# iamsonderr/icl-mixed-precision-gmres

Hardware: AMD Instinct MI355X
Metric: GMRES iterations/sec + SpMV achieved HBM GB/s, 10M-nnz CSR, 1/2/4/8 GPUs (higher is better)
Workload: dtype f32; 1 GPU; BAND banded CSR n=1000000, offsets -5..+4, nnz=9999975 (1e6 rows = 10M nnz per GPU, 1 GPU(s)); GMRES(30) mixed (fp32 Arnoldi, f32 accumulation, fp64 residual/update), cgs, identity preconditioner, tol=0; step=one restart cycle = 30 iterations, rows_per_gpu=1000000, nnz=9999975, parallelism=one GPU

## Files before the change

### icl-mixed-precision-gmres_amd/__init__.py

```python
from __future__ import annotations

import ctypes as C
import os
import subprocess
from dataclasses import dataclass, field
from pathlib import Path
from typing import Optional

import numpy as np

from ._abi import (ACCUMS, ENGINES, MODES, ORTHS, PRECS, SPMV_FORMATS, STATUS, ArnoldiDesc, CondestResult, CyclePolicy, HostCsr, RankLayout, SolveArgs,
                   SolveResult, condest_args, condest_dict)

PKG_DIR = Path(__file__).resolve().parent
REPO_DIR = PKG_DIR.parent
LIB_DIR = PKG_DIR / "lib"
HIP_LIB = LIB_DIR / "libmpgmres_hip.so"
HOST_LIB = LIB_DIR / "libmpgmres_host.so"
CLI = PKG_DIR / "bin" / "gmres_perf_test"


def build(jobs: int = 8) -> None:
    subprocess.run(["make", "-C", str(PKG_DIR), f"-j{jobs}"], check=True)

# ... 128 lines not shown
    lib.mpg_halo_recv_count.argtypes = [C.c_void_p, _I32]
    lib.mpg_halo_recv_count.restype = _I32
    lib.mpg_halo_recv_rows.argtypes = [C.c_void_p, _I32, P64]
    lib.mpg_halo_set_send.argtypes = [C.c_void_p, _I32, _I32, P64]
    lib.mpg_halo_local_cols.argtypes = [C.c_void_p, P32]
    lib.mpg_halo_free.argtypes = [C.c_void_p]
    lib.mpg_halo_free.restype = None
    lib.mpg_rccl_unique_id.argtypes = [C.c_char_p, C.c_int]
    lib.mpg_engine_create_dist.argtypes = [C.POINTER(SolveArgs), C.c_void_p, C.c_char_p, _I32, _I32,
                                           C.POINTER(C.c_void_p), C.c_char_p, C.c_int]
    lib.mpg_solve_loopback.argtypes = [C.POINTER(SolveArgs), _I32, C.POINTER(SolveResult)]
    lib.mpg_solve_loopback_ex.argtypes = [C.POINTER(SolveArgs), _I32, C.POINTER(SolveResult), C.c_void_p]
    lib.mpg_solve_multi_gpu.argtypes = [C.POINTER(SolveArgs), _I32, C.c_void_p, C.POINTER(SolveResult), C.c_void_p]
    lib.mpg_engine_comm_ranks.argtypes = [C.c_void_p]
    lib.mpg_engine_sell_columns.argtypes = [C.c_void_p, C.POINTER(C.c_int32), C.POINTER(C.c_int64),
                                            C.POINTER(C.c_int64)]
    lib.mpg_engine_half_stats.argtypes = [C.c_void_p, C.POINTER(C.c_int64)]
    lib.mpg_engine_slices_per_wave.argtypes = [C.c_void_p]
    lib.mpg_engine_givens_folded.argtypes = [C.c_void_p]
    lib.mpg_engine_step_dots_steps.argtypes = [C.c_void_p]
    lib.mpg_engine_step_dots_status.argtypes = [C.c_void_p, C.c_int]
    lib.mpg_engine_givens_rider.argtypes = [C.c_void_p]
    lib.mpg_engine_cgs_stream_steps.argtypes = [C.c_void_p]
    lib.mpg_engine_tail_fold.argtypes = [C.c_void_p]
    lib.mpg_engine_cycle_policy.argtypes = [C.c_void_p, C.POINTER(CyclePolicy)]
    lib.mpg_cycle_plan_describe.argtypes = [C.POINTER(CyclePolicy), C.c_char_p, C.c_int]
    lib.mpg_engine_accum.argtypes = [C.c_void_p]
    lib.mpg_engine_basis.argtypes = [C.c_void_p]
    lib.mpg_engine_prec_fused.argtypes = [C.c_void_p]
    lib.mpg_engine_prec_sweeps.argtypes = [C.c_void_p]
    lib.mpg_engine_prec_interval.argtypes = [C.c_void_p, C.POINTER(C.c_double), C.POINTER(C.c_double)]
    lib.mpg_cheb_coeffs.argtypes = [C.c_int, C.c_double, C.c_double, C.POINTER(C.c_double), C.POINTER(C.c_double)]
    lib.mpg_engine_prec_roots.argtypes = [C.c_void_p, C.POINTER(C.c_double), C.POINTER(C.c_double), C.c_int32]
    lib.mpg_gmres_poly_roots.argtypes = [C.c_int, C.POINTER(C.c_double), C.c_int, C.POINTER(C.c_double),
                                         C.POINTER(C.c_double), C.POINTER(C.c_int)]
    lib.mpg_engine_prologue_format.argtypes = [C.c_void_p]
    lib.mpg_engine_sell_shared_slices.argtypes = [C.c_void_p]
    lib.mpg_engine_sell_shared_slices.restype = C.c_int64
    lib.mpg_engine_sell_sigma.argtypes = [C.c_void_p]
    lib.mpg_solve_from.argtypes = [C.POINTER(SolveArgs), C.c_void_p, C.POINTER(SolveResult)]
    lib.mpg_solve_from.restype = C.c_int
    lib.mpg_engine_rearm.argtypes = [C.c_void_p, C.c_void_p, C.c_void_p, C.c_void_p, C.c_int]
    lib.mpg_engine_x.argtypes = [C.c_void_p, C.c_void_p, C.c_int]
    lib.mpg_engine_solves.argtypes = [C.c_void_p]
    lib.mpg_engine_graph_captures.argtypes = [C.c_void_p]

# ... 774 lines not shown
        per = (C.c_double * cap)()
        which = {"spmv": 0, "cgs_update": 2, "dots": 3}[phase]
        cnt = self._lib.mpg_engine_time_phase_stamps(self._h, which, reps, C.byref(ms), per, cap)
        if cnt < 0:
            msg = self._lib.mpg_engine_last_error(self._h).decode(errors="replace")
            raise RuntimeError(f"mpg_engine_time_phase_stamps failed ({cnt}): {msg}")
        return ms.value, [per[i] for i in range(min(cnt, cap))]

    def phase_bytes(self, phase: str) -> float:
        return float(self._lib.mpg_engine_phase_bytes(self._h, self.PHASES[phase]))

    def spmv_layout(self) -> dict:
        f, w, cb, st, win = C.c_int32(), C.c_int32(), C.c_int32(), C.c_int64(), C.c_int32()
        if self._lib.mpg_engine_spmv_layout(self._h, C.byref(f), C.byref(w), C.byref(cb), C.byref(st), C.byref(win)):
            raise RuntimeError("mpg_engine_spmv_layout failed")
        fused = int(self._lib.mpg_engine_step_dots_steps(self._h))
        pf = int(self._lib.mpg_engine_prec_fused(self._h))
        ps = int(self._lib.mpg_engine_prec_sweeps(self._h))
        ia, ib = C.c_double(), C.c_double()
        has_iv = self._lib.mpg_engine_prec_interval(self._h, C.byref(ia), C.byref(ib)) == 0
        rre, rim = (C.c_double * 64)(), (C.c_double * 64)()
        nroots = int(self._lib.mpg_engine_prec_roots(self._h, rre, rim, 64))
        stream = int(self._lib.mpg_engine_cgs_stream_steps(self._h))
        rider = int(self._lib.mpg_engine_givens_rider(self._h)) == 1
        tail = int(self._lib.mpg_engine_tail_fold(self._h)) == 1
        basis = int(self._lib.mpg_engine_basis(self._h))
        return _Layout({**({"dots_fused": fused} if fused > 0 else {}), **({"givens_rider": True} if rider else {}),
                **({"tail_fold": True} if tail else {}),
                **({"cgs_stream": stream} if stream > 0 else {}), "format": {1: "csr", 2: "sell", 3: "node"}[f.value], "vec_width": w.value, "col_bytes": cb.value,
                "stored": st.value, "window": bool(win.value),
                "slices_per_wave": int(self._lib.mpg_engine_slices_per_wave(self._h)),
                "givens_folded": bool(self._lib.mpg_engine_givens_folded(self._h) == 1),
                "accum": {0: "f64", 1: "f32"}[int(self._lib.mpg_engine_accum(self._h))],
                **({"basis": {1: "f16", 2: "f16emu"}[basis]} if basis else {}),
                **({"prec_fused": pf} if pf >= 0 else {}),
                **({"prec_sweeps": ps} if ps >= 0 else {}),
                **({"prec_interval": (ia.value, ib.value)} if has_iv else {}),
                **({"prec_roots": [complex(rre[i], rim[i]) for i in range(nroots)]} if nroots >= 0 else {}),
                "prologue": {1: "csr", 2: "sell", 3: "node"}[int(self._lib.mpg_engine_prologue_format(self._h))]})

    def step_dots_status(self, k: int) -> int:
        return int(self._lib.mpg_engine_step_dots_status(self._h, k))

    def cycle_policy(self) -> CyclePolicy:
        p = CyclePolicy()
        if self._lib.mpg_engine_cycle_policy(self._h, C.byref(p)):
            raise RuntimeError("mpg_engine_cycle_policy failed")
        return p

    def sell_columns(self) -> dict:
# ... 28 lines not shown
```

### icl-mixed-precision-gmres_amd/csrc/arnoldi.hip

```cpp
#include "arnoldi_launch.hpp"

#include <cstdlib>
#include <new>
#include <algorithm>
#include <vector>

using namespace mpg;

namespace {

int64_t sell_copy_bytes(const mpg_arnoldi* a);

void node_prologue_build(mpg_arnoldi* a) {
    const char* e = std::getenv("MPG_NODE_PROLOGUE");
    if ((e && *e == '0') || a->node.nblk == 0 || a->d.n_front != 0 || a->d.outer_type != MPG_F64) return;
    if (hipMalloc((void**)&a->rsum, (size_t)std::max(a->d.n, 1) * sizeof(double)) != hipSuccess) {
        (void)hipGetLastError();
        return;
    }
    if (a->d.val_outer == a->d.val_inner && a->d.inner_val == MPG_F64) {
        a->node_res = &a->node;
        return;
    }
    const int64_t csr = a->d.A->nnz * 12 + ((int64_t)a->d.n + 1) * 4;
// ... 52 lines not shown
}

}

extern "C" {

int mpg_arnoldi_create(mpg_ctx_t ctx, const mpg_arnoldi_desc* desc, mpg_arnoldi_t* out) {
    if (!ctx || !desc || !out || !desc->A || desc->n < 0 || desc->n_ext < desc->n || desc->m < 1 ||
        desc->m > 1000 || desc->orth < 0 || desc->orth > 2)
        return MPG_ERR_ARG;
    *out = nullptr;
    int combo = combo_of(*desc);
    if (combo < 0) return MPG_ERR_UNSUPPORTED;
    if (desc->A->rows != desc->n || desc->A->cols > desc->n_ext) return MPG_ERR_ARG;
    if (desc->inner_row_exp && desc->inner_val != MPG_F16) return MPG_ERR_ARG;
    if (desc->block_dinv && (desc->jacobi || desc->prec_block < 2 || desc->prec_block > 4)) return MPG_ERR_ARG;
    mpg_arnoldi* a = new (std::nothrow) mpg_arnoldi();
    if (!a) return MPG_ERR_ALLOC;
    a->ctx = ctx;
    a->d = *desc;
    a->combo = combo;
    a->tsize = desc->vec_type == MPG_F64 ? 8 : 4;
    if (const char* e = std::getenv("MPG_CGS_PREFETCH"); e && (*e == '0' || *e == '1')) a->cgs_pref = *e - '0';
    a->G = desc->A->nblocks < kGroups ? (desc->A->nblocks > 0 ? desc->A->nblocks : 1) : kGroups;
    a->Grb = desc->A->nblocks > 0 ? desc->A->nblocks : 1;
    a->Gd = (int)std::min<int64_t>(kCombineGroups, std::max<int64_t>(1, ((int64_t)desc->n + 4 * kCombineBlock - 1) /
                                                                          (4 * kCombineBlock)));
    if (desc->n_front < 0) {
        delete a;
        return MPG_ERR_ARG;
    }
    a->front = MPG_FRONT_PAD(desc->n_front);
    const size_t align = 256 / a->tsize;
    a->ld = ((int64_t)desc->n + align - 1) / align * align;
    if (a->ld == 0) a->ld = align;
    const int m = desc->m;
    auto alloc = [&](void** p, size_t bytes) {
        if (hipMalloc(p, bytes ? bytes : 16) != hipSuccess) return false;
        return hipMemsetAsync(*p, 0, bytes ? bytes : 16, ctx->stream) == hipSuccess;
    };
    bool ok = alloc(&a->V, (size_t)a->ld * (m + 1) * a->tsize) && alloc(&a->H, (size_t)(m + 1) * m * a->tsize) &&
              alloc(&a->small, (size_t)7 * (m + 1) * a->tsize) &&
              alloc(&a->wbase[0], (size_t)(a->front + desc->n_ext + 64) * a->tsize) &&
              alloc(&a->wbase[1], (size_t)(a->front + desc->n_ext + 64) * a->tsize) &&
              alloc((void**)&a->partial, std::max<size_t>(std::max<size_t>((size_t)(kNC + 4) * a->Grb,
                                                                           (size_t)(m + 4) * a->G),
// ... 188 lines not shown
        else
            k_prologue_finish_parts<T, X, 1024><<<1, 1024, 0, a->ctx->stream>>>(
                a->last_G, a->last_part, a->sums, m, static_cast<T*>(a->s()), static_cast<T*>(a->inv()), a->report,
                stage, hcol);
        return MPG_OK;
    });
    if (st) return st;
    a->tail_staged = false;
    MPG_LAUNCH_CHECK(a->ctx);
    return MPG_OK;
}

int mpg_arnoldi_reduce(mpg_arnoldi_t a, int ncols) { return phases(a).reduce(a, ncols); }

int mpg_arnoldi_spmv(mpg_arnoldi_t a, int k) { return phases(a).spmv(a, k, 0, false); }
int mpg_arnoldi_spmv_dots(mpg_arnoldi_t a, int k, int fold) {
    if (fold < 0 || fold > 2) return MPG_ERR_ARG;
    return phases(a).spmv(a, k, fold, true);
}
int mpg_arnoldi_spmv_dots_supported(mpg_arnoldi_t a, int k) { return phases(a).spmv_dots_ok(a, k); }
int mpg_arnoldi_step_dots(mpg_arnoldi_t a, int k, int fold) { return phases(a).step_dots(a, k, fold); }
int mpg_arnoldi_step_dots_supported(mpg_arnoldi_t a, int k) { return phases(a).step_dots_ok(a, k); }
int mpg_arnoldi_cgs_stream_at(mpg_arnoldi_t a, int k) { return phases(a).cgs_stream_at(a, k); }
int mpg_arnoldi_givens_spmv(mpg_arnoldi_t a, int k) { return phases(a).spmv(a, k, 1, false); }
int mpg_arnoldi_givens_partials_spmv(mpg_arnoldi_t a, int k) { return phases(a).spmv(a, k, 2, false); }
int mpg_arnoldi_fold_max_m(void) { return kFoldMaxM; }
int mpg_arnoldi_partials_max_cols(void) { return kWideMax; }

constexpr int kFoldMaxGroups = 4096;
int mpg_arnoldi_fold_pays(mpg_arnoldi_t a) {
    if (!a) return 0;
    const char* env = std::getenv("MPG_FOLD_MAX_GROUPS");
    const int64_t limit = env && *env ? std::atoll(env) : kFoldMaxGroups;
    if (a->node.nblk > 0) {
        const int tpw = node_tpw(a->node);
        return (a->node.ntiles + tpw - 1) / tpw <= limit ? 1 : 0;
    }
    const SellCopy& S = a->sell;
    if (S.nslices == 0) return a->Grb <= limit ? 1 : 0;
    const int per_group = (kStepSellBlock / kWave) * (sell_uniform(S) && sell_pair(S) ? 2 : 1);
    return (S.nslices + per_group - 1) / per_group <= limit ? 1 : 0;
}

int mpg_arnoldi_dots(mpg_arnoldi_t a, int k) { return phases(a).dots(a, k, false); }
int mpg_arnoldi_dots_sums(mpg_arnoldi_t a, int k) { return phases(a).dots(a, k, true); }

// ... 110 lines not shown
```

### icl-mixed-precision-gmres_amd/csrc/arnoldi_dots.hpp

```cpp
#pragma once

#include "arnoldi_spmv.hpp"

namespace {

template <class T, int BS = kBlock, bool COMBINE = false, class A = double>
__global__ __launch_bounds__(BS) void k_panel_dots(int n, const T* __restrict__ V, int64_t ld, int c0, int nc,
                                                   const T* __restrict__ w, double* __restrict__ partial,
                                                   unsigned* __restrict__ cnt, double* __restrict__ sums) {
    A acc[kNC];
#pragma unroll
    for (int c = 0; c < kNC; ++c) acc[c] = A(0);
    const int n4 = n & ~3;
    const T* __restrict__ Vb = V + (int64_t)c0 * ld;
    for (int i = 4 * (blockIdx.x * BS + threadIdx.x); i < n4; i += 4 * gridDim.x * BS) {
        A wv[4];
        Row4<T>::load(w + i, wv);
#pragma unroll
        for (int c = 0; c < kNC; ++c) {
            if (c < nc) {
                A v[4];
                Row4<T>::load(Vb + (int64_t)c * ld + i, v);
                acc[c] += v[0] * wv[0] + v[1] * wv[1] + v[2] * wv[2] + v[3] * wv[3];
            }
        }
// ... 64 lines not shown
        }
    }
    store_partials<NP, BS>(acc, NC, partial, G);
}

template <class T, int BS, int NC, class A = double, class BT = T>
__device__ __forceinline__ void dots_panel(int n, const typename Basis<T, BT>::elem* __restrict__ V, int64_t ld,
                                           const T* __restrict__ w, double* __restrict__ partial) {
    dots_panel_from<T, BS, NC, A, BT>(n, V, ld, DotsGlobal<T, A, BT>{w, {}}, partial);
}

template <class T, int BS, int NC, bool STAMP = false, class AT = double>
__global__ __launch_bounds__(BS) void k_dots_nc(int n, const T* __restrict__ V, int64_t ld,
                                                const T* __restrict__ w, double* __restrict__ partial,
                                                unsigned long long* stamp) {
    using A = typename AccOf<AT>::type;
    using Bs = BasisOf<T, AT>;
    stamp_at<STAMP>(stamp, 0);
    dots_panel<T, BS, NC, A, typename AccOf<AT>::template basis<T>>(n, basis_ptr<Bs>(V), ld, w, partial);
    stamp_at<STAMP>(stamp, 1);
}

constexpr int kStepDotsRows = 4 * kCombineBlock;

template <class T, class A, int HELD>
struct DotsStaged {
    static constexpr bool kStaged = true;
    static constexpr int kHeld = HELD;
    const T* wst;
    const T* vkst;
    int base;
    Raw4<T> held[HELD > 0 ? HELD : 1];
    __device__ __forceinline__ void load_w(int i, A (&wv)[4]) const { Row4<T>::load(wst + (i - base), wv); }
    __device__ __forceinline__ Raw4<T> newest(int i) const {
        Raw4<T> r;
        r.load(vkst + (i - base));
        return r;
    }
};

__device__ __forceinline__ void wave_lds_handoff() {
    __atomic_signal_fence(__ATOMIC_SEQ_CST);
    __builtin_amdgcn_s_waitcnt(0xC07F);
    wave_lds_sync();
    __atomic_signal_fence(__ATOMIC_SEQ_CST);
}

template <class T, class P, int W, bool FOLD, int BE, int NC, bool PF, class A>
__global__ __launch_bounds__(kCombineBlock) void k_step_dots(int n, int nslices, const int16_t* __restrict__ col,
                                                             const T* __restrict__ val, const T* __restrict__ wprev,
                                                             const T* __restrict__ inv_p, T* __restrict__ V,
                                                             int64_t ld, int k, const P* __restrict__ diag,
                                                             T* __restrict__ w, GivensFold<T> fold,
                                                             const int32_t* __restrict__ spat,
                                                             const int64_t* __restrict__ coff,
                                                             const int16_t* __restrict__ pat, int64_t ustride,
                                                             double* __restrict__ dpart) {
    static_assert(std::is_same_v<T, float>, "fp32 basis and values");
    using CI = int16_t;
    using Row = SellRow<T, CI, W, (MPG_SELL_NT != 0), BE>;
    constexpr int BS = kCombineBlock, SPW = 4, NW = BS / kWave;
    constexpr int RB = kStepDotsRows, RW = SPW * kWave;
    constexpr int WL = kWinLo + RW + kWinHi;
    static_assert(NW * RW == RB, "four slices per wave cover the workgroup's rows");
    static_assert(RW == 4 * kWave, "a wave's slices are its lanes' row groups of dots_panel_from");
    __shared__ __attribute__((aligned(16))) T win[NW][WL];
    __shared__ __attribute__((aligned(16))) T wst[RB];
    const int tid = threadIdx.x, lane = tid & (kWave - 1), wid = wave_id();
    constexpr int NG = kBlock / kWave;
    if constexpr (FOLD) {
        if (blockIdx.x == gridDim.x - 1) {
// ... 20 lines not shown
    if constexpr (FOLD) fold_parts_load(fold, lane, part);
    __builtin_amdgcn_sched_barrier(0);
    const int i4 = base + 4 * tid;
    const bool in4 = i4 < n;
    Raw4<T> wr;
    wr.load(wprev + (in4 ? i4 : 0));
    const int clo = row0 - kWinLo + lane, chi = row0 + RW + lane;
    const bool lo_in = clo >= 0 && clo < n, hi_in = chi < n;
    const T wlo = wprev[lo_in ? clo : 0];
    const T whi = wprev[hi_in ? chi : 0];
    __builtin_amdgcn_sched_barrier(0);
#pragma unroll
    for (int p = 0; p < SPW; ++p) {
        row[p].init_vals(lane, val);
        row[p].load_vals(0);
    }
    __builtin_amdgcn_sched_barrier(0);
#pragma unroll
    for (int p = 0; p < SPW; ++p) {
        row[p].init_finish(lane, col, val, nullptr, pat);
        row[p].load_cols(0);
    }
    __builtin_amdgcn_sched_barrier(0);
    constexpr int B = kColBatch<T>;
    constexpr int HMAX = FOLD ? 6 : B;
    constexpr int HELD = !PF ? 0 : NC - 1 < HMAX ? NC - 1 : HMAX;
    T* const wwin = win[wid];
    DotsStaged<T, A, HELD> src;
    src.wst = wst + wid * RW;
    src.vkst = wwin + kWinLo;
    src.base = row0;
    if constexpr (HELD > 0) {
#pragma unroll
        for (int u = 0; u < HELD; ++u) src.held[u].load(V + (int64_t)u * ld + (in4 ? i4 : 0));
    }
    __builtin_amdgcn_sched_barrier(0);
    T inv;
    if constexpr (FOLD) inv = inv_of_norm2<T>(fold_parts_sum(fold, part));
    else inv = *inv_p;
    {
        T vq[4];
#pragma unroll
        for (int r = 0; r < 4; ++r) vq[r] = in4 ? (T)(wr.template at<T>(r) * inv) : T(0);
        Row4<T>::store(wwin + kWinLo + 4 * lane, vq);
        wwin[lane] = lo_in ? (T)(wlo * inv) : T(0);
        wwin[kWinLo + RW + lane] = hi_in ? (T)(whi * inv) : T(0);
    }
    wave_lds_handoff();
    auto xv = [&](int c) { return (double)wwin[c - row0 + kWinLo]; };
    A sum[SPW] = {};
#pragma unroll
    for (int p = 0; p < SPW; ++p)
        if (live_p[p]) row[p].sum(0, xv, sum[p]);
#pragma unroll
    for (int p = 0; p < SPW; ++p) {
        if (live_p[p])
            for (int q = Row::U; q < row[p].steps; q += Row::U) {
                row[p].load(q);
                row[p].sum(q, xv, sum[p]);
            }
        const int i = (s0 + p) * kWave + lane;
        T wi = T(0);
        if (live_p[p] && i < n) {
            const T t = (T)sum[p];
            wi = precond<T, P>(t, diag, i);
            w[i] = wi;
            V[(int64_t)k * ld + i] = wwin[i - row0 + kWinLo];
        }
        wst[i - base] = wi;
    }
    wave_lds_handoff();
    dots_panel_from<T, BS, NC, A>(n, V, ld, src, dpart, G);
}

template <class T, int BS, int NCL, class A = double>
__global__ __launch_bounds__(BS) void k_dots_panels(int n, const T* __restrict__ V, int64_t ld,
                                                    const T* __restrict__ w, double* __restrict__ partial) {
    const int c0 = blockIdx.y * kNC;
    double* __restrict__ part = partial + (size_t)c0 * gridDim.x;
    if (blockIdx.y + 1 < gridDim.y) dots_panel<T, BS, kNC, A>(n, V + (int64_t)c0 * ld, ld, w, part);
    else dots_panel<T, BS, NCL, A>(n, V + (int64_t)c0 * ld, ld, w, part);
}

}
```

### icl-mixed-precision-gmres_amd/csrc/arnoldi_launch.hpp

```cpp
#pragma once

#include "arnoldi_dots.hpp"
#include "arnoldi_orth.hpp"
#include "arnoldi_update.hpp"

#include <algorithm>
#include <cstdlib>
#include <tuple>
#include <type_traits>

namespace {

template <class A, class F>
int dispatch_acc(int combo, F&& f) {
    if constexpr (std::is_same_v<A, double>) {
        return dispatch(combo, f);
    } else {
        switch (combo) {
            case 2: return f(float(), float(), float(), float());
            case 3: return f(float(), double(), float(), float());
            case 4: return f(float(), double(), float(), half_v());
            default: return MPG_ERR_UNSUPPORTED;
        }
    }
// ... 195 lines not shown
    if (st) return st;
    if (dots) {
        a->last_G = a->fd_ng;
        a->last_part = a->dpart;
    }
    MPG_LAUNCH_CHECK(a->ctx);
    return MPG_OK;
}

template <class A>
int step_dots_check(const mpg_arnoldi* a, int k) {
    if (!a || k < 0 || k >= a->d.m) return MPG_ERR_ARG;
    const SellCopy& S = a->sell;
    const bool ok = std::is_same_v<A, float> && (a->combo == 2 || a->combo == 3) && plain_basis(a) &&
                    a->d.orth != kOrthMGS && a->d.orth != kOrthCGSR && k + 1 <= kNC &&
                    a->d.n > 0 && a->d.n % 4 == 0 &&
                    (int64_t)a->Gd * kStepDotsRows >= a->d.n &&
                    a->front == 0 && a->d.n_ext == a->d.n &&
                    S.nslices > 0 && S.c16 && S.win && !S.rows && sell_uniform(S) && S.W == 2 &&
                    S.ustride / kWave <= 10;
    return ok ? MPG_OK : MPG_ERR_UNSUPPORTED;
}

template <class A>
int step_dots_run(mpg_arnoldi_t a, int k, int fold) {
    if (!a || k < 0 || k >= a->d.m || fold < 0 || fold > 2) return MPG_ERR_ARG;
    if (int st = step_dots_check<A>(a, k)) return st;
    if (fold && (k < 1 || a->d.m > kFoldMaxM)) return MPG_ERR_ARG;
    if constexpr (std::is_same_v<A, float>) {
        using T = float;
        using P = float;
        const bool again = fold == 2 && a->sd_k == k && a->last_part == a->dpart;
        if (fold == 2 && !again) {
            a->sd_k = k;
            a->sd_part = a->last_part;
            a->sd_G = a->last_G;
        }
        if (fold == 2 && (a->sd_G > kBlock || a->sd_part == a->dpart)) return MPG_ERR_ARG;
        GivensFold<T> gf{nullptr, 0, {}};
        if (fold) gf = GivensFold<T>{fold == 2 ? a->sd_part : a->sums, fold == 2 ? a->sd_G : 0, givens_args<T>(a, k - 1)};
        const SellCopy& S = a->sell;
        const P* diag = a->d.jacobi ? static_cast<const P*>(a->d.diag) : nullptr;
        int st = with_nc<kNC>(k + 1, [&](auto nc) {
            constexpr int NC = decltype(nc)::value;
            return with_flag(fold, [&](auto fo) {
                launch_timed(a->ctx, k_step_dots<T, P, 2, decltype(fo)::value, 10, NC, true, A>,
                             dim3(a->Gd + (fold ? 1 : 0)), dim3(kCombineBlock), a->d.n, S.nslices,
                             static_cast<const int16_t*>(S.col), static_cast<const T*>(S.val),
                             static_cast<const T*>(a->w[k & 1]), static_cast<const T*>(a->inv()),
                             static_cast<T*>(a->V), a->ld, k, diag, static_cast<T*>(a->w[(k + 1) & 1]), gf, S.spat,
                             S.coff, static_cast<const int16_t*>(S.pat), S.ustride, a->dpart);
                return (int)MPG_OK;
            });
        });
        if (st) return st;
        a->last_G = a->Gd;
        a->last_part = a->dpart;
        MPG_LAUNCH_CHECK(a->ctx);
        return MPG_OK;
    } else {
        return MPG_ERR_UNSUPPORTED;
    }
}

inline int wide_groups(const mpg_arnoldi* a, int ncols) {
    const int np = (ncols + kNC - 1) / kNC;
    return std::max(1, std::min(a->Gd, kCombineGroups / np));
}

inline unsigned long long* take_stamp(mpg_arnoldi* a, int64_t waves) {
    unsigned long long* p = a->ctx->stamp_next;
    a->ctx->stamp_next = nullptr;
    return p && waves <= a->ctx->stamp_cap ? p : nullptr;
}

// ... 314 lines not shown
                constexpr bool SNAP = decltype(snap)::value;
                k_update_tail_nc<T, X, decltype(nc)::value, A, stream, SNAP><<<a->Gd, kCombineBlock, 0, a->ctx->stream>>>(
                    a->d.n, static_cast<const T*>(a->V), a->ld, static_cast<X*>(a->d.x),
                    SNAP ? static_cast<X*>(a->x_snap) : nullptr, tl);
                return (int)MPG_OK;
            });
        });
    });
    if (st) return st;
    a->tail_staged = true;
    MPG_LAUNCH_CHECK(a->ctx);
    return MPG_OK;
}

}

struct mpg_arnoldi_phases {
    int (*reduce)(mpg_arnoldi* a, int ncols);
    int (*spmv)(mpg_arnoldi* a, int k, int fold, bool dots);
    int (*step_dots)(mpg_arnoldi* a, int k, int fold);
    int (*step_dots_ok)(const mpg_arnoldi* a, int k);
    int (*spmv_dots_ok)(const mpg_arnoldi* a, int k);
    int (*cgs_stream_at)(const mpg_arnoldi* a, int k);
    int (*dots)(mpg_arnoldi* a, int k, bool combine);
    int (*cgs)(mpg_arnoldi* a, int k, int pass, bool givens, bool from_partials, bool no_next);
    int (*mgs)(mpg_arnoldi* a, int k, int j, bool from_partials);
    int (*givens)(mpg_arnoldi* a, int k, bool from_partials);
    int (*update)(mpg_arnoldi* a, int k);
    int (*update_tail)(mpg_arnoldi* a, int m, int flags);
};
__attribute__((visibility("hidden"))) const mpg_arnoldi_phases& mpg_arnoldi_phases_acc32();

namespace {
template <class A>
mpg_arnoldi_phases phases_of() {
    return {reduce_run<A>, spmv_run<A>,     step_dots_run<A>, step_dots_check<A>, spmv_dots_check<A>, cgs_stream_check<A>,
            dots_run<A>,   cgs_run<A>,      mgs_run<A>,       givens_run<A>,      update_run<A>,      update_tail_run<A>};
}
}
```

### icl-mixed-precision-gmres_amd/csrc/arnoldi_plan.hpp

```cpp
#pragma once

#include "internal.hpp"
#include "node_tile.hpp"
#include "sell_tile.hpp"
#include "mpgmres/arnoldi.h"

#include <algorithm>
#include <cstdlib>
#include <type_traits>

using namespace mpg;

namespace {

constexpr int kNC = 32;
constexpr int kGroups = 1024;
constexpr int kCombineBlock = 1024;
constexpr int kCombineGroups = 256;
constexpr int kOrthMGS = 1, kOrthCGSR = 2;
constexpr int kFoldMaxM = 128;
constexpr int kWideMax = 128;

template <int C, int N, class F>
__device__ __forceinline__ void static_for(F&& f) {
// ... 33 lines not shown
struct mpg_arnoldi {
    mpg_ctx* ctx = nullptr;
    mpg_arnoldi_desc d{};
    int combo = 0;
    int G = 1;
    int Grb = 1;
    int last_G = 1;
    double* last_part = nullptr;
    int64_t ld = 0;
    size_t tsize = 8;
    void* V = nullptr;
    void* H = nullptr;
    void* small = nullptr;
    void* w[2] = {nullptr, nullptr};
    void* wbase[2] = {nullptr, nullptr};
    int front = 0;
    double* partial = nullptr;
    double* dpart = nullptr;
    double* sums = nullptr;
    double* report = nullptr;
    unsigned* counters = nullptr;
    int Gd = 1;
    int cgs_pref = -1;
    SellCopy sell;
    SellCopy sell_outer;
    NodeCopy node;
    NodeCopy node_outer;
    const NodeCopy* node_res = nullptr;
    double* rsum = nullptr;
    bool outer_is_inner = false;
    double* fd_part = nullptr;
    unsigned* fd_cnt = nullptr;
    int fd_gs = 0, fd_ng = 0;
    int sd_k = -1, sd_G = 0;
    double* sd_part = nullptr;
    bool acc32 = false;
    int basis = 0;
    void* x_snap = nullptr;
    bool tail_staged = false;

    char* small_at(int slot) const { return static_cast<char*>(small) + (size_t)slot * (d.m + 1) * tsize; }
    void* cs() const { return small_at(0); }
    void* sn() const { return small_at(1); }
    void* s() const { return small_at(2); }
    void* corr() const { return small_at(3); }
    void* inv() const { return small_at(4); }
// ... 50 lines not shown
```

### icl-mixed-precision-gmres_amd/csrc/lds_ring.hpp

```cpp
#pragma once

#include "internal.hpp"

namespace {

typedef __attribute__((address_space(3))) void* lds_ptr_t;
typedef float f32x4_t __attribute__((ext_vector_type(4)));
constexpr int kStreamSlots = 9;

__device__ __forceinline__ double cgs_stream_load_partial(const double* p) {
    double v;
    asm volatile("global_load_dwordx2 %0, %1, off" : "=v"(v) : "v"(p) : "memory");
    return v;
}
template <int BEHIND>
__device__ __forceinline__ void cgs_stream_wait_partials(double (&p)[8]) {
    asm volatile("s_waitcnt vmcnt(%8)"
                 : "+v"(p[0]), "+v"(p[1]), "+v"(p[2]), "+v"(p[3]), "+v"(p[4]), "+v"(p[5]), "+v"(p[6]), "+v"(p[7])
                 : "i"(BEHIND)
                 : "memory");
    __builtin_amdgcn_sched_barrier(0);
}
template <int BEHIND>
__device__ __forceinline__ void cgs_stream_take(unsigned slot_lds, unsigned coef_lds, f32x4_t& v, float& cu) {
    asm volatile("s_waitcnt vmcnt(%4)\n\tds_read_b128 %0, %2\n\tds_read_b32 %1, %3\n\ts_waitcnt lgkmcnt(0)"
                 : "=&v"(v), "=&v"(cu)
                 : "v"(slot_lds), "v"(coef_lds), "i"(BEHIND)
                 : "memory");
    __builtin_amdgcn_sched_barrier(0);
}
__device__ __forceinline__ void cgs_stream_request(const float* g, unsigned lds_wave) {
    __builtin_amdgcn_global_load_lds(g, (lds_ptr_t)(size_t)lds_wave, 16, 0, 0);
}
__device__ __forceinline__ void cgs_stream_pin(float (&t)[4]) {
    asm volatile("" : "+v"(t[0]), "+v"(t[1]), "+v"(t[2]), "+v"(t[3]));
}

}
```

### icl-mixed-precision-gmres_amd/host/fused_gmres.cpp

```cpp
#include "fused_gmres.hpp"

#include <algorithm>
#include <chrono>
#include <cmath>
#include <cstdio>
#include <cstring>
#include <functional>
#include <stdexcept>
#include <thread>

#include "gmres.hpp"
#include "types_hip.hpp"

namespace mpg {

DevMem::DevMem(mpg_ctx_t c, size_t b) : ctx(c), bytes(b) { check(mpg_malloc(c, b, &p), "mpg_malloc", c); }
DevMem::~DevMem() {
    if (p) mpg_free(ctx, p);
}
DevMem& DevMem::operator=(DevMem&& o) noexcept {
    if (this != &o) {
        if (p) mpg_free(ctx, p);
        ctx = o.ctx;
        p = o.p;
// ... 1013 lines not shown
    }
    return p_->poly_roots.count;
}
bool FusedEngine::prec_interval(double* a, double* b) const {
    if (!p_->cheb) return false;
    if (a) *a = p_->cheb_iv.a;
    if (b) *b = p_->cheb_iv.b;
    return true;
}
int FusedEngine::step_dots_steps() const {
    return (int)std::count_if(p_->cycle.begin(), p_->cycle.end(), [](const Op& o) { return o.kind == OpKind::StepDots; });
}
bool FusedEngine::givens_rider() const {
    return std::any_of(p_->cycle.begin(), p_->cycle.end(), [](const Op& o) { return o.kind == OpKind::StepDots && o.b != 0; });
}
bool FusedEngine::tail_fold() const {
    return std::any_of(p_->cycle.begin(), p_->cycle.end(), [](const Op& o) { return o.kind == OpKind::GivensUpdate; });
}
int FusedEngine::cgs_stream_steps() const {
    return (int)std::count_if(p_->cycle.begin(), p_->cycle.end(), [&](const Op& o) {
        return o.kind == OpKind::CgsPartials && mpg_arnoldi_cgs_stream_at(p_->arn, o.a) == 1;
    });
}
const CyclePolicy& FusedEngine::policy() const { return p_->pol; }
const std::vector<Op>& FusedEngine::cycle_ops() const { return p_->cycle; }
hipStream_t FusedEngine::stream() const { return p_->stream(); }
mpg_ctx_t FusedEngine::ctx() const { return p_->ctx; }

void fill_history(const FusedEngine& e, mpg_solve_result* r) {
    r->status = e.status;
    r->restarts = e.restarts;
    r->inner_k = e.inner_k;
    r->total_iters = (int64_t)e.total_iters();
    r->minvb_norm = e.minvb_norm;
    r->setup_seconds = e.setup_seconds;
    r->n_cycles = (int64_t)e.cycles.size();
    for (size_t c = 0; c < e.cycles.size() && (int64_t)c < r->cycle_cap; ++c) {
        if (r->cyc_r_norm) r->cyc_r_norm[c] = e.cycles[c].r_norm;
        if (r->cyc_normalization) r->cyc_normalization[c] = e.cycles[c].normalization;
        if (r->cyc_beta) r->cyc_beta[c] = e.cycles[c].beta;
    }
    r->nonfinite_steps = e.breakdown.steps;
    r->nonfinite_cycles = e.breakdown.cycles;
    r->first_nonfinite_step = e.breakdown.first_step;
    r->n_steps = (int64_t)e.step_res.size();
    for (size_t s = 0; s < e.step_res.size() && (int64_t)s < r->step_cap; ++s) {
// ... 129 lines not shown
int mpg_engine_prologue_format(mpg_engine_t e) {
    if (!e || !e->eng) return MPG_ERR_ARG;
    return mpg_arnoldi_prologue_format(e->eng->arnoldi());
}

int mpg_engine_givens_folded(mpg_engine_t e) {
    if (!e || !e->eng) return MPG_ERR_ARG;
    return e->eng->policy().fold;
}

int mpg_engine_step_dots_steps(mpg_engine_t e) {
    if (!e || !e->eng) return MPG_ERR_ARG;
    return e->eng->step_dots_steps();
}

int mpg_engine_givens_rider(mpg_engine_t e) {
    if (!e || !e->eng) return MPG_ERR_ARG;
    return e->eng->givens_rider() ? 1 : 0;
}

int mpg_engine_tail_fold(mpg_engine_t e) {
    return e && e->eng ? (e->eng->tail_fold() ? 1 : 0) : -1;
}
int mpg_engine_cgs_stream_steps(mpg_engine_t e) {
    if (!e || !e->eng) return MPG_ERR_ARG;
    return e->eng->cgs_stream_steps();
}

int mpg_engine_cycle_policy(mpg_engine_t e, mpg_cycle_policy* out) {
    if (!e || !e->eng || !out) return MPG_ERR_ARG;
    *out = e->eng->policy();
    return MPG_OK;
}

int mpg_engine_step_dots_status(mpg_engine_t e, int k) {
    if (!e || !e->eng) return MPG_ERR_ARG;
    return mpg_arnoldi_step_dots_supported(e->eng->arnoldi(), k);
}

int mpg_engine_comm_ranks(mpg_engine_t e) {
    if (!e || !e->eng) return MPG_ERR_ARG;
    return e->comm ? e->comm->transport_ranks() : 1;
}

int64_t mpg_engine_sell_shared_slices(mpg_engine_t e) {
    if (!e || !e->eng) return MPG_ERR_ARG;
// ... 35 lines not shown
```

### icl-mixed-precision-gmres_amd/host/fused_gmres.hpp

```cpp
#ifndef MPGMRES_FUSED_GMRES_HPP
#define MPGMRES_FUSED_GMRES_HPP

#include <hip/hip_runtime.h>

#include <functional>
#include <memory>
#include <stdexcept>
#include <string>
#include <vector>

#include "IterUtil.hpp"
#include "cycle_plan.hpp"
#include "mpgmres/arnoldi.h"
#include "mpgmres/capi.h"
#include "mpgmres/solve.h"
#include "types_hip.hpp"

namespace mpg {

inline void check_sweep_prec_args(const mpg_solve_args& a, const std::string& name) {
    if (a.jacobi_steps < 1 || a.jacobi_steps > 64)
        throw std::invalid_argument("prec " + name + ": jacobi_steps = " + std::to_string(a.jacobi_steps) +
                                    " is outside [1, 64]");
    if (a.mode == MPG_MODE_SINGLE_PREC)
// ... 70 lines not shown

    int run(int max_cycles, bool& done);
    void finish_report(mpg_solve_result* r);

    void rearm(const double* b, const double* x0, const double* x_true, int flags);
    void copy_x(double* dst, bool dst_on_device);
    int solves() const { return solves_; }
    int graph_captures() const { return graph_captures_; }

    size_t total_iters() const { return conv_->total_iterations(); }
    double time_phase(int which, int reps, bool inplace = false, std::vector<double>* per_launch = nullptr);
    double time_phase_graph(int which, int reps, std::vector<double>* per_launch = nullptr);
    double time_phase_stamps(int which, int reps, std::vector<double>* per_launch = nullptr);
    double time_phase_dup(int which, int reps, int64_t* launches = nullptr, bool step_dots_only = false);
    double phase_bytes(int which) const;
    mpg_arnoldi_t arnoldi() const;
    int basis() const;
    const int64_t* half_stats() const;
    int prec_fused() const;
    int prec_sweeps() const;
    bool prec_interval(double* a, double* b) const;
    int prec_roots(double* re, double* im, int cap) const;
    int cgs_stream_steps() const;
    int step_dots_steps() const;
    bool givens_rider() const;
    bool tail_fold() const;
    void sync();
    const CyclePolicy& policy() const;

    std::vector<CycleRecord> cycles;
    std::vector<double> step_res;
    std::vector<int> step_cycle;
    int status = 0;
    int64_t restarts = 0;
    int64_t inner_k = 0;
    double minvb_norm = 0, b_norm = 0, a_norm = 0;
    double setup_seconds = 0;
    BreakdownLog breakdown;
    bool measured = false;

private:
    struct Impl;
    std::unique_ptr<Impl> p_;
    std::unique_ptr<Convergence<double, void>> conv_;
    int solves_ = 0, graph_captures_ = 0;
    void arm(const double* b, const double* x0, const double* x_true, int flags);
// ... 52 lines not shown
```

### include/mpgmres/arnoldi.h

```cpp
#ifndef MPGMRES_ARNOLDI_H
#define MPGMRES_ARNOLDI_H

#include <stdint.h>

#include "mpgmres/capi.h"

#ifdef __cplusplus
extern "C" {
#endif

typedef enum { MPG_F64 = 0, MPG_F32 = 1, MPG_F16 = 2 } mpg_dtype_t;

typedef struct mpg_arnoldi* mpg_arnoldi_t;

typedef struct {
    int32_t n;
    int32_t n_ext;
    int32_t m;
    int32_t orth;
    int32_t vec_type;
    int32_t outer_type;
    int32_t prec_type;
    int32_t inner_val;
    int32_t jacobi;
// ... 32 lines not shown
int mpg_arnoldi_prologue(mpg_arnoldi_t a);
int mpg_arnoldi_prologue_finish(mpg_arnoldi_t a);
int mpg_arnoldi_prologue_finish_partials(mpg_arnoldi_t a);
int mpg_arnoldi_prologue_wnorm(mpg_arnoldi_t a);
int mpg_arnoldi_spmv(mpg_arnoldi_t a, int k);
int mpg_arnoldi_dots(mpg_arnoldi_t a, int k);
int mpg_arnoldi_cgs(mpg_arnoldi_t a, int k, int pass);
int mpg_arnoldi_cgs_partials(mpg_arnoldi_t a, int k);
int mpg_arnoldi_partials_max_cols(void);
int mpg_arnoldi_cgsr_wide_pass(mpg_arnoldi_t a, int k, int pass);
int mpg_arnoldi_mgs(mpg_arnoldi_t a, int k, int j);
int mpg_arnoldi_mgs_partials(mpg_arnoldi_t a, int k, int j);
int mpg_arnoldi_givens(mpg_arnoldi_t a, int k);
int mpg_arnoldi_givens_partials(mpg_arnoldi_t a, int k);
int mpg_arnoldi_givens_spmv(mpg_arnoldi_t a, int k);
int mpg_arnoldi_dots_sums(mpg_arnoldi_t a, int k);
int mpg_arnoldi_cgs_givens(mpg_arnoldi_t a, int k, int pass);
int mpg_arnoldi_givens_partials_spmv(mpg_arnoldi_t a, int k);
int mpg_arnoldi_spmv_dots(mpg_arnoldi_t a, int k, int fold);
int mpg_arnoldi_spmv_dots_supported(mpg_arnoldi_t a, int k);
int mpg_arnoldi_step_dots(mpg_arnoldi_t a, int k, int fold);
int mpg_arnoldi_step_dots_supported(mpg_arnoldi_t a, int k);
int mpg_arnoldi_cgs_stream_at(mpg_arnoldi_t a, int k);
int mpg_arnoldi_fold_max_m(void);
int mpg_arnoldi_fold_pays(mpg_arnoldi_t a);
int mpg_arnoldi_update(mpg_arnoldi_t a, int k);
int mpg_arnoldi_update_tail(mpg_arnoldi_t a, int m, int flags);
int mpg_arnoldi_update_tail_supported(mpg_arnoldi_t a);
int mpg_arnoldi_set_x_snapshot(mpg_arnoldi_t a, void* x_snap);
int mpg_arnoldi_reduce(mpg_arnoldi_t a, int ncols);

double* mpg_arnoldi_sums_dev(mpg_arnoldi_t a);
void* mpg_arnoldi_wprev_dev(mpg_arnoldi_t a, int k);
int mpg_arnoldi_vec_bytes(mpg_arnoldi_t a);
const double* mpg_arnoldi_report_dev(mpg_arnoldi_t a);
int mpg_arnoldi_report_len(mpg_arnoldi_t a);
const void* mpg_arnoldi_basis_dev(mpg_arnoldi_t a, int64_t* ld);
const void* mpg_arnoldi_hessenberg_dev(mpg_arnoldi_t a);
const void* mpg_arnoldi_inv_dev(mpg_arnoldi_t a);
const void* mpg_arnoldi_rotations_dev(mpg_arnoldi_t a, int which);
int mpg_arnoldi_time_next_spmv(mpg_arnoldi_t a, void* start_event, void* stop_event);
int mpg_arnoldi_stamp_next(mpg_arnoldi_t a, unsigned long long* slots, int64_t cap_waves);
int64_t mpg_arnoldi_stamp_waves(mpg_arnoldi_t a);

int mpg_arnoldi_num_groups(mpg_arnoldi_t a);

// ... 22 lines not shown
```

### include/mpgmres/solve.h

```cpp
#ifndef MPGMRES_SOLVE_H
#define MPGMRES_SOLVE_H

#include <stddef.h>
#include <stdint.h>

#ifdef __cplusplus
extern "C" {
#endif

typedef enum {
    MPG_MODE_MIXED = 0,
    MPG_MODE_BASELINE = 1,
    MPG_MODE_SINGLE_PREC = 2,
    MPG_MODE_SINGLE = 3,
    MPG_MODE_MIXED_HALF = 4
} mpg_mode_t;

typedef enum { MPG_ORTH_CGS = 0, MPG_ORTH_MGS = 1, MPG_ORTH_CGSR = 2 } mpg_orth_t;

typedef enum {
    MPG_PREC_ILU = 0,
    MPG_PREC_ILU_JACOBI = 1,
    MPG_PREC_JACOBI = 2,
    MPG_PREC_IDENTITY = 3,
// ... 75 lines not shown
int mpg_engine_graph_captures(mpg_engine_t e);
int mpg_engine_sync(mpg_engine_t e);
int64_t mpg_engine_total_iters(mpg_engine_t e);
int mpg_engine_report(mpg_engine_t e, mpg_solve_result* result);
int mpg_engine_time_phase(mpg_engine_t e, int which, int reps, double* avg_ms);
int mpg_engine_time_spmv_incycle(mpg_engine_t e, int cycles, double* avg_ms, double* per_launch_ms, int cap);
int mpg_engine_time_phase_dup(mpg_engine_t e, int which, int reps, double* avg_ms, int64_t* launches);
int mpg_engine_time_phase_stamps(mpg_engine_t e, int which, int reps, double* avg_ms, double* per_launch_ms,
                                 int cap);
int mpg_engine_time_phase_graph(mpg_engine_t e, int which, int reps, double* avg_ms, double* per_launch_ms,
                                int cap);
double mpg_engine_phase_bytes(mpg_engine_t e, int which);
int mpg_engine_spmv_layout(mpg_engine_t e, int32_t* format, int32_t* vec_width, int32_t* col_bytes,
                           int64_t* stored, int32_t* window);
int mpg_engine_sell_columns(mpg_engine_t e, int32_t* form, int64_t* csr_slices, int64_t* implicit_slices);
int64_t mpg_engine_sell_shared_slices(mpg_engine_t e);
int mpg_engine_sell_sigma(mpg_engine_t e);
int mpg_engine_givens_folded(mpg_engine_t e);
int mpg_engine_step_dots_steps(mpg_engine_t e);
int mpg_engine_step_dots_status(mpg_engine_t e, int k);
int mpg_engine_givens_rider(mpg_engine_t e);
int mpg_engine_tail_fold(mpg_engine_t e);
int mpg_engine_cgs_stream_steps(mpg_engine_t e);
int mpg_engine_prec_fused(mpg_engine_t e);
int mpg_engine_prec_sweeps(mpg_engine_t e);
int mpg_engine_prec_interval(mpg_engine_t e, double* a, double* b);
int mpg_cheb_coeffs(int steps, double theta, double delta, double* alpha, double* beta);
int mpg_engine_prec_roots(mpg_engine_t e, double* re, double* im, int32_t cap);
int mpg_gmres_poly_roots(int s, const double* H, int ldh, double* re, double* im, int* count);
int mpg_engine_accum(mpg_engine_t e);
int mpg_engine_basis(mpg_engine_t e);
int mpg_engine_prologue_format(mpg_engine_t e);
int mpg_engine_comm_ranks(mpg_engine_t e);
int mpg_engine_slices_per_wave(mpg_engine_t e);
int mpg_engine_half_stats(mpg_engine_t e, int64_t* stats);
int mpg_engine_destroy(mpg_engine_t e);

#define MPG_CYCLE_POLICY_STEPS 128
typedef struct {
    int32_t ranks;
    int32_t orth;
    int32_t m;
    int32_t graph;
    int32_t pipeline;
    int32_t fold;
    int32_t combine;
// ... 27 lines not shown
```

Baseline: 30620 GMRES iterations/s.

## Stream earlier basis columns through an LDS ring in fused step-dots kernel

Adds a RING variant of the fused SpMV+dots step kernel. For steps with more earlier basis columns than the register-held batch, it prefetches those columns straight from global memory into an LDS ring with asynchronous global_load_lds. It then consumes them with explicit vmcnt waits, overlapping the loads with the dot-product accumulation instead of using the plain panel path. It is on by default for steps k>=7 (env MPG_STEP_RING can force it on or off), and adds a query for how many steps use it. In exchange it uses more LDS per block, which may lower occupancy, and relies on hand-written inline asm for the wait counts.

Result: slower. 30300 GMRES iterations/s (-1.0%).

```diff
diff --git a/icl-mixed-precision-gmres_amd/__init__.py b/icl-mixed-precision-gmres_amd/__init__.py
--- a/icl-mixed-precision-gmres_amd/__init__.py
+++ b/icl-mixed-precision-gmres_amd/__init__.py
@@ -174,6 +174,7 @@
     lib.mpg_engine_step_dots_status.argtypes = [C.c_void_p, C.c_int]
     lib.mpg_engine_givens_rider.argtypes = [C.c_void_p]
     lib.mpg_engine_cgs_stream_steps.argtypes = [C.c_void_p]
+    lib.mpg_engine_step_ring_steps.argtypes = [C.c_void_p]
     lib.mpg_engine_tail_fold.argtypes = [C.c_void_p]
     lib.mpg_engine_cycle_policy.argtypes = [C.c_void_p, C.POINTER(CyclePolicy)]
     lib.mpg_cycle_plan_describe.argtypes = [C.POINTER(CyclePolicy), C.c_char_p, C.c_int]
@@ -994,10 +995,12 @@
         rre, rim = (C.c_double * 64)(), (C.c_double * 64)()
         nroots = int(self._lib.mpg_engine_prec_roots(self._h, rre, rim, 64))
         stream = int(self._lib.mpg_engine_cgs_stream_steps(self._h))
+        ring = int(self._lib.mpg_engine_step_ring_steps(self._h))
         rider = int(self._lib.mpg_engine_givens_rider(self._h)) == 1
         tail = int(self._lib.mpg_engine_tail_fold(self._h)) == 1
         basis = int(self._lib.mpg_engine_basis(self._h))
         return _Layout({**({"dots_fused": fused} if fused > 0 else {}), **({"givens_rider": True} if rider else {}),
+                **({"step_ring": ring} if ring > 0 else {}),
                 **({"tail_fold": True} if tail else {}),
                 **({"cgs_stream": stream} if stream > 0 else {}), "format": {1: "csr", 2: "sell", 3: "node"}[f.value], "vec_width": w.value, "col_bytes": cb.value,
                 "stored": st.value, "window": bool(win.value),
diff --git a/icl-mixed-precision-gmres_amd/csrc/arnoldi.hip b/icl-mixed-precision-gmres_amd/csrc/arnoldi.hip
--- a/icl-mixed-precision-gmres_amd/csrc/arnoldi.hip
+++ b/icl-mixed-precision-gmres_amd/csrc/arnoldi.hip
@@ -98,6 +98,7 @@
     a->combo = combo;
     a->tsize = desc->vec_type == MPG_F64 ? 8 : 4;
     if (const char* e = std::getenv("MPG_CGS_PREFETCH"); e && (*e == '0' || *e == '1')) a->cgs_pref = *e - '0';
+    if (const char* e = std::getenv("MPG_STEP_RING"); e && (*e == '0' || *e == '1')) a->step_ring = *e - '0';
     a->G = desc->A->nblocks < kGroups ? (desc->A->nblocks > 0 ? desc->A->nblocks : 1) : kGroups;
     a->Grb = desc->A->nblocks > 0 ? desc->A->nblocks : 1;
     a->Gd = (int)std::min<int64_t>(kCombineGroups, std::max<int64_t>(1, ((int64_t)desc->n + 4 * kCombineBlock - 1) /
@@ -332,6 +333,7 @@
 int mpg_arnoldi_step_dots(mpg_arnoldi_t a, int k, int fold) { return phases(a).step_dots(a, k, fold); }
 int mpg_arnoldi_step_dots_supported(mpg_arnoldi_t a, int k) { return phases(a).step_dots_ok(a, k); }
 int mpg_arnoldi_cgs_stream_at(mpg_arnoldi_t a, int k) { return phases(a).cgs_stream_at(a, k); }
+int mpg_arnoldi_step_ring_at(mpg_arnoldi_t a, int k, int fold) { return phases(a).step_ring_at(a, k, fold); }
 int mpg_arnoldi_givens_spmv(mpg_arnoldi_t a, int k) { return phases(a).spmv(a, k, 1, false); }
 int mpg_arnoldi_givens_partials_spmv(mpg_arnoldi_t a, int k) { return phases(a).spmv(a, k, 2, false); }
 int mpg_arnoldi_fold_max_m(void) { return kFoldMaxM; }
diff --git a/icl-mixed-precision-gmres_amd/csrc/arnoldi_dots.hpp b/icl-mixed-precision-gmres_amd/csrc/arnoldi_dots.hpp
--- a/icl-mixed-precision-gmres_amd/csrc/arnoldi_dots.hpp
+++ b/icl-mixed-precision-gmres_amd/csrc/arnoldi_dots.hpp
@@ -1,6 +1,7 @@
 #pragma once
 
 #include "arnoldi_spmv.hpp"
+#include "lds_ring.hpp"
 
 namespace {
 
@@ -111,6 +112,8 @@
 }
 
 constexpr int kStepDotsRows = 4 * kCombineBlock;
+template <bool FOLD>
+constexpr int kStepHeldMax = FOLD ? 6 : kColBatch<float>;
 
 template <class T, class A, int HELD>
 struct DotsStaged {
@@ -135,7 +138,7 @@
     __atomic_signal_fence(__ATOMIC_SEQ_CST);
 }
 
-template <class T, class P, int W, bool FOLD, int BE, int NC, bool PF, class A>
+template <class T, class P, int W, bool FOLD, int BE, int NC, bool PF, class A, bool RING = false>
 __global__ __launch_bounds__(kCombineBlock) void k_step_dots(int n, int nslices, const int16_t* __restrict__ col,
                                                              const T* __restrict__ val, const T* __restrict__ wprev,
                                                              const T* __restrict__ inv_p, T* __restrict__ V,
@@ -202,8 +205,7 @@
         row[p].load_cols(0);
     }
     __builtin_amdgcn_sched_barrier(0);
-    constexpr int B = kColBatch<T>;
-    constexpr int HMAX = FOLD ? 6 : B;
+    constexpr int HMAX = kStepHeldMax<FOLD>;
     constexpr int HELD = !PF ? 0 : NC - 1 < HMAX ? NC - 1 : HMAX;
     T* const wwin = win[wid];
     DotsStaged<T, A, HELD> src;
@@ -232,25 +234,107 @@
 #pragma unroll
     for (int p = 0; p < SPW; ++p)
         if (live_p[p]) row[p].sum(0, xv, sum[p]);
-#pragma unroll
-    for (int p = 0; p < SPW; ++p) {
-        if (live_p[p])
-            for (int q = Row::U; q < row[p].steps; q += Row::U) {
-                row[p].load(q);
-                row[p].sum(q, xv, sum[p]);
+    if constexpr (RING) {
+        static_assert(PF && NC - 1 > HMAX && HELD == HMAX, "more earlier columns than the held batch");
+        static_assert(sizeof(T) == 4 && sizeof(A) == 4, "the ring holds an fp32 basis for fp32 sums");
+        constexpr int M = NC - 1 - HELD;
+        constexpr int R = M < kStepRingSlots ? M : kStepRingSlots;
+        constexpr int NP = Pow2Ceil<NC>::v;
+        __shared__ float4 ring[R][BS];
+        static_assert(sizeof(float4) == 16 && sizeof(ring[0]) == 16 * BS && BS % kWave == 0 &&
+                          sizeof(ring) + sizeof(win) + sizeof(wst) + 3 * sizeof(T) * (kFoldMaxM + 2) +
+                                  sizeof(A) * NW * NP + 64 <=
+                              160 * 1024,
+                      "lane-linear 16-B image, whole waves, inside the CU's LDS");
+        T wo[SPW], vo[SPW];
+#pragma unroll
+        for (int p = 0; p < SPW; ++p) {
+            if (live_p[p])
+                for (int q = Row::U; q < row[p].steps; q += Row::U) {
+                    row[p].load(q);
+                    row[p].sum(q, xv, sum[p]);
+                }
+            const int i = (s0 + p) * kWave + lane;
+            T wi = T(0);
+            if (live_p[p] && i < n) wi = precond<T, P>((T)sum[p], diag, i);
+            wo[p] = wi;
+            vo[p] = wwin[i - row0 + kWinLo];
+            wst[i - base] = wi;
+        }
+        wave_lds_handoff();
+#pragma unroll
+        for (int p = 0; p < SPW; ++p) asm volatile("" : "+v"(wo[p]), "+v"(vo[p]));
+        __builtin_amdgcn_s_waitcnt(0x0F70);
+        __builtin_amdgcn_sched_barrier(0);
+#pragma unroll
+        for (int p = 0; p < SPW; ++p) {
+            const int i = (s0 + p) * kWave + lane;
+            if (live_p[p] && i < n) {
+                w[i] = wo[p];
+                V[(int64_t)k * ld + i] = vo[p];
             }
-        const int i = (s0 + p) * kWave + lane;
-        T wi = T(0);
-        if (live_p[p] && i < n) {
-            const T t = (T)sum[p];
-            wi = precond<T, P>(t, diag, i);
-            w[i] = wi;
-            V[(int64_t)k * ld + i] = wwin[i - row0 + kWinLo];
-        }
-        wst[i - base] = wi;
-    }
-    wave_lds_handoff();
-    dots_panel_from<T, BS, NC, A>(n, V, ld, src, dpart, G);
+        }
+        __builtin_amdgcn_sched_barrier(0);
+        const int ip = in4 ? i4 : 0;
+        const unsigned ring_lane = (unsigned)(size_t)(lds_ptr_t)&ring[0][tid];
+        const unsigned ring_wave = __builtin_amdgcn_readfirstlane(ring_lane);
+        const T* Vr = V + (int64_t)HELD * ld + ip;
+#pragma unroll
+        for (int u = 0; u < R; ++u) cgs_stream_request(Vr + (int64_t)u * ld, ring_wave + u * 16 * BS);
+        __builtin_amdgcn_sched_barrier(0);
+        f32x4_t wq, nq;
+        ring_read_pair((unsigned)(size_t)(lds_ptr_t)(wst + wid * RW + 4 * lane),
+                       (unsigned)(size_t)(lds_ptr_t)(wwin + kWinLo + 4 * lane), wq, nq);
+        const A wv[4] = {(A)wq.x, (A)wq.y, (A)wq.z, (A)wq.w};
+        A acc[NP];
+#pragma unroll
+        for (int c = 0; c < NP; ++c) acc[c] = A(0);
+        auto add = [&](A& a, const Raw4<T>& v) {
+            const A e = v.template at<A>(0) * wv[0] + v.template at<A>(1) * wv[1] + v.template at<A>(2) * wv[2] +
+                        v.template at<A>(3) * wv[3];
+            a += in4 ? e : A(0);
+        };
+#pragma unroll
+        for (int c = 0; c < HELD; ++c) add(acc[c], src.held[c]);
+        {
+            Raw4<T> v;
+            v.v = make_float4(nq.x, nq.y, nq.z, nq.w);
+            add(acc[NC - 1], v);
+        }
+        static_for<0, M>([&](auto jj) {
+            constexpr int j = decltype(jj)::value;
+            constexpr unsigned slot = (unsigned)((j % R) * 16 * BS);
+            constexpr int behind = M - 1 - j < R - 1 ? M - 1 - j : R - 1;
+            f32x4_t q;
+            ring_take<behind>(ring_lane + slot, q);
+            if constexpr (j + R < M) cgs_stream_request(Vr + (int64_t)(j + R) * ld, ring_wave + slot);
+            Raw4<T> v;
+            v.v = make_float4(q.x, q.y, q.z, q.w);
+            add(acc[HELD + j], v);
+            asm volatile("" : "+v"(acc[HELD + j]));
+        });
+        store_partials<NP, BS>(acc, NC, dpart, G);
+    } else {
+#pragma unroll
+        for (int p = 0; p < SPW; ++p) {
+            if (live_p[p])
+                for (int q = Row::U; q < row[p].steps; q += Row::U) {
+                    row[p].load(q);
+                    row[p].sum(q, xv, sum[p]);
+                }
+            const int i = (s0 + p) * kWave + lane;
+            T wi = T(0);
+            if (live_p[p] && i < n) {
+                const T t = (T)sum[p];
+                wi = precond<T, P>(t, diag, i);
+                w[i] = wi;
+                V[(int64_t)k * ld + i] = wwin[i - row0 + kWinLo];
+            }
+            wst[i - base] = wi;
+        }
+        wave_lds_handoff();
+        dots_panel_from<T, BS, NC, A>(n, V, ld, src, dpart, G);
+    }
 }
 
 template <class T, int BS, int NCL, class A = double>
diff --git a/icl-mixed-precision-gmres_amd/csrc/arnoldi_launch.hpp b/icl-mixed-precision-gmres_amd/csrc/arnoldi_launch.hpp
--- a/icl-mixed-precision-gmres_amd/csrc/arnoldi_launch.hpp
+++ b/icl-mixed-precision-gmres_amd/csrc/arnoldi_launch.hpp
@@ -241,6 +241,21 @@
     return ok ? MPG_OK : MPG_ERR_UNSUPPORTED;
 }
 
+constexpr int kStepRingFrom = 7;
+inline bool step_ring_form(const mpg_arnoldi* a, int k, bool fold) {
+    const bool built = k > (fold ? kStepHeldMax<true> : kStepHeldMax<false>);
+    if (!built || a->step_ring == 0) return false;
+    return a->step_ring == 1 || k >= kStepRingFrom;
+}
+
+template <class A>
+int step_ring_check(const mpg_arnoldi* a, int k, int fold) {
+    if (!a || k < 0 || k >= a->d.m || fold < 0 || fold > 2) return MPG_ERR_ARG;
+    if (!plain_basis(a)) return MPG_ERR_UNSUPPORTED;
+    if (step_dots_check<A>(a, k) != MPG_OK) return 0;
+    return step_ring_form(a, k, fold != 0);
+}
+
 template <class A>
 int step_dots_run(mpg_arnoldi_t a, int k, int fold) {
     if (!a || k < 0 || k >= a->d.m || fold < 0 || fold > 2) return MPG_ERR_ARG;
@@ -263,13 +278,19 @@
         int st = with_nc<kNC>(k + 1, [&](auto nc) {
             constexpr int NC = decltype(nc)::value;
             return with_flag(fold, [&](auto fo) {
-                launch_timed(a->ctx, k_step_dots<T, P, 2, decltype(fo)::value, 10, NC, true, A>,
-                             dim3(a->Gd + (fold ? 1 : 0)), dim3(kCombineBlock), a->d.n, S.nslices,
-                             static_cast<const int16_t*>(S.col), static_cast<const T*>(S.val),
-                             static_cast<const T*>(a->w[k & 1]), static_cast<const T*>(a->inv()),
-                             static_cast<T*>(a->V), a->ld, k, diag, static_cast<T*>(a->w[(k + 1) & 1]), gf, S.spat,
-                             S.coff, static_cast<const int16_t*>(S.pat), S.ustride, a->dpart);
-                return (int)MPG_OK;
+                constexpr bool FOLD = decltype(fo)::value;
+                auto go = [&](auto kern) {
+                    launch_timed(a->ctx, kern, dim3(a->Gd + (fold ? 1 : 0)), dim3(kCombineBlock), a->d.n, S.nslices,
+                                 static_cast<const int16_t*>(S.col), static_cast<const T*>(S.val),
+                                 static_cast<const T*>(a->w[k & 1]), static_cast<const T*>(a->inv()),
+                                 static_cast<T*>(a->V), a->ld, k, diag, static_cast<T*>(a->w[(k + 1) & 1]), gf, S.spat,
+                                 S.coff, static_cast<const int16_t*>(S.pat), S.ustride, a->dpart);
+                    return (int)MPG_OK;
+                };
+                if constexpr (NC - 1 > kStepHeldMax<FOLD>) {
+                    if (step_ring_form(a, k, FOLD)) return go(k_step_dots<T, P, 2, FOLD, 10, NC, true, A, true>);
+                }
+                return go(k_step_dots<T, P, 2, FOLD, 10, NC, true, A>);
             });
         });
         if (st) return st;
@@ -630,6 +651,7 @@
     int (*step_dots_ok)(const mpg_arnoldi* a, int k);
     int (*spmv_dots_ok)(const mpg_arnoldi* a, int k);
     int (*cgs_stream_at)(const mpg_arnoldi* a, int k);
+    int (*step_ring_at)(const mpg_arnoldi* a, int k, int fold);
     int (*dots)(mpg_arnoldi* a, int k, bool combine);
     int (*cgs)(mpg_arnoldi* a, int k, int pass, bool givens, bool from_partials, bool no_next);
     int (*mgs)(mpg_arnoldi* a, int k, int j, bool from_partials);
@@ -643,6 +665,7 @@
 template <class A>
 mpg_arnoldi_phases phases_of() {
     return {reduce_run<A>, spmv_run<A>,     step_dots_run<A>, step_dots_check<A>, spmv_dots_check<A>, cgs_stream_check<A>,
+            step_ring_check<A>,
             dots_run<A>,   cgs_run<A>,      mgs_run<A>,       givens_run<A>,      update_run<A>,      update_tail_run<A>};
 }
 }
diff --git a/icl-mixed-precision-gmres_amd/csrc/arnoldi_plan.hpp b/icl-mixed-precision-gmres_amd/csrc/arnoldi_plan.hpp
--- a/icl-mixed-precision-gmres_amd/csrc/arnoldi_plan.hpp
+++ b/icl-mixed-precision-gmres_amd/csrc/arnoldi_plan.hpp
@@ -79,6 +79,7 @@
     unsigned* counters = nullptr;
     int Gd = 1;
     int cgs_pref = -1;
+    int step_ring = -1;
     SellCopy sell;
     SellCopy sell_outer;
     NodeCopy node;
diff --git a/icl-mixed-precision-gmres_amd/csrc/lds_ring.hpp b/icl-mixed-precision-gmres_amd/csrc/lds_ring.hpp
--- a/icl-mixed-precision-gmres_amd/csrc/lds_ring.hpp
+++ b/icl-mixed-precision-gmres_amd/csrc/lds_ring.hpp
@@ -7,6 +7,7 @@
 typedef __attribute__((address_space(3))) void* lds_ptr_t;
 typedef float f32x4_t __attribute__((ext_vector_type(4)));
 constexpr int kStreamSlots = 9;
+constexpr int kStepRingSlots = 7;
 
 __device__ __forceinline__ double cgs_stream_load_partial(const double* p) {
     double v;
@@ -29,6 +30,21 @@
                  : "memory");
     __builtin_amdgcn_sched_barrier(0);
 }
+template <int BEHIND>
+__device__ __forceinline__ void ring_take(unsigned slot_lds, f32x4_t& v) {
+    asm volatile("s_waitcnt vmcnt(%2)\n\tds_read_b128 %0, %1\n\ts_waitcnt lgkmcnt(0)"
+                 : "=&v"(v)
+                 : "v"(slot_lds), "i"(BEHIND)
+                 : "memory");
+    __builtin_amdgcn_sched_barrier(0);
+}
+__device__ __forceinline__ void ring_read_pair(unsigned a_lds, unsigned b_lds, f32x4_t& a, f32x4_t& b) {
+    asm volatile("ds_read_b128 %0, %2\n\tds_read_b128 %1, %3\n\ts_waitcnt lgkmcnt(0)"
+                 : "=&v"(a), "=&v"(b)
+                 : "v"(a_lds), "v"(b_lds)
+                 : "memory");
+    __builtin_amdgcn_sched_barrier(0);
+}
 __device__ __forceinline__ void cgs_stream_request(const float* g, unsigned lds_wave) {
     __builtin_amdgcn_global_load_lds(g, (lds_ptr_t)(size_t)lds_wave, 16, 0, 0);
 }
diff --git a/icl-mixed-precision-gmres_amd/host/fused_gmres.cpp b/icl-mixed-precision-gmres_amd/host/fused_gmres.cpp
--- a/icl-mixed-precision-gmres_amd/host/fused_gmres.cpp
+++ b/icl-mixed-precision-gmres_amd/host/fused_gmres.cpp
@@ -1059,6 +1059,11 @@
         return o.kind == OpKind::CgsPartials && mpg_arnoldi_cgs_stream_at(p_->arn, o.a) == 1;
     });
 }
+int FusedEngine::step_ring_steps() const {
+    return (int)std::count_if(p_->cycle.begin(), p_->cycle.end(), [&](const Op& o) {
+        return o.kind == OpKind::StepDots && mpg_arnoldi_step_ring_at(p_->arn, o.a, o.b) == 1;
+    });
+}
 const CyclePolicy& FusedEngine::policy() const { return p_->pol; }
 const std::vector<Op>& FusedEngine::cycle_ops() const { return p_->cycle; }
 hipStream_t FusedEngine::stream() const { return p_->stream(); }
@@ -1234,6 +1239,10 @@
 int mpg_engine_tail_fold(mpg_engine_t e) {
     return e && e->eng ? (e->eng->tail_fold() ? 1 : 0) : -1;
 }
+int mpg_engine_step_ring_steps(mpg_engine_t e) {
+    if (!e) return MPG_ERR_ARG;
+    return e->eng->step_ring_steps();
+}
 int mpg_engine_cgs_stream_steps(mpg_engine_t e) {
     if (!e || !e->eng) return MPG_ERR_ARG;
     return e->eng->cgs_stream_steps();
diff --git a/icl-mixed-precision-gmres_amd/host/fused_gmres.hpp b/icl-mixed-precision-gmres_amd/host/fused_gmres.hpp
--- a/icl-mixed-precision-gmres_amd/host/fused_gmres.hpp
+++ b/icl-mixed-precision-gmres_amd/host/fused_gmres.hpp
@@ -116,6 +116,7 @@
     bool prec_interval(double* a, double* b) const;
     int prec_roots(double* re, double* im, int cap) const;
     int cgs_stream_steps() const;
+    int step_ring_steps() const;
     int step_dots_steps() const;
     bool givens_rider() const;
     bool tail_fold() const;
diff --git a/include/mpgmres/arnoldi.h b/include/mpgmres/arnoldi.h
--- a/include/mpgmres/arnoldi.h
+++ b/include/mpgmres/arnoldi.h
@@ -78,6 +78,7 @@
 int mpg_arnoldi_step_dots(mpg_arnoldi_t a, int k, int fold);
 int mpg_arnoldi_step_dots_supported(mpg_arnoldi_t a, int k);
 int mpg_arnoldi_cgs_stream_at(mpg_arnoldi_t a, int k);
+int mpg_arnoldi_step_ring_at(mpg_arnoldi_t a, int k, int fold);
 int mpg_arnoldi_fold_max_m(void);
 int mpg_arnoldi_fold_pays(mpg_arnoldi_t a);
 int mpg_arnoldi_update(mpg_arnoldi_t a, int k);
diff --git a/include/mpgmres/solve.h b/include/mpgmres/solve.h
--- a/include/mpgmres/solve.h
+++ b/include/mpgmres/solve.h
@@ -121,6 +121,7 @@
 int mpg_engine_givens_rider(mpg_engine_t e);
 int mpg_engine_tail_fold(mpg_engine_t e);
 int mpg_engine_cgs_stream_steps(mpg_engine_t e);
+int mpg_engine_step_ring_steps(mpg_engine_t e);
 int mpg_engine_prec_fused(mpg_engine_t e);
 int mpg_engine_prec_sweeps(mpg_engine_t e);
 int mpg_engine_prec_interval(mpg_engine_t e, double* a, double* b);
```
